# Rintazero/ft8_demodulator

Measured on AMD Instinct MI355X. Metric: 15-s FT8 slots/sec (full decode) + LDPC candidates/sec, 1/2/4/8 MI355X, higher is better.
Workload: dtype f32 (STFT, sync score) / f64 (LLR, BP); 1 GPU; BASELINE config 3: batch of 256 independent 15-s slots per GPU, 12 kHz, K=300 candidates, min_score=2, 20 BP iterations (config 5 shape at N>1); slots_per_gpu=256, max_candidates=300, min_score=2, pipeline_depth=2, parallelism=slot-sharded x1

## Files before the change

ft8_demodulator_amd/csrc/bp.hip:

```cpp
#include "ft8_internal.h"
#include "heap_replay.h"

namespace ft8 {
namespace {

__constant__ uint16_t kChkStartD[FT8_LDPC_M + 1] = FT8_CHK_START_INIT;
__constant__ uint8_t kEdgeVarD[FT8_LDPC_E] = FT8_EDGE_VAR_INIT;
__constant__ uint16_t kVarEdgeD[FT8_LDPC_N * 3] = FT8_VAR_EDGE_INIT;
__constant__ uint8_t kEdgeChkD[FT8_LDPC_E] = FT8_EDGE_CHK_INIT;
constexpr int kGrayD[8] = {0, 1, 3, 2, 5, 6, 4, 7};

constexpr int kEdgeSlots = (FT8_LDPC_E + kWave - 1) / kWave;
constexpr int kVarSlots = (FT8_LDPC_N + kWave - 1) / kWave;
constexpr int kChkSlots = (FT8_LDPC_M + kWave - 1) / kWave;

constexpr int kDivGroup = 3;
static_assert(kEdgeSlots % kDivGroup == 0 && kVarSlots == kDivGroup, "division groups tile the slots exactly");
constexpr int kBpWavesPerSimd = 4;
constexpr int kBpLbWaves = 3;
constexpr int kBpGridCus = 256;
constexpr double kClip2 = 2.0 * 4.97;

typedef __attribute__((address_space(3))) const double lds_f64;
typedef __attribute__((address_space(3))) const uint64_t lds_u64;

__device__ double sqrt_rn(double x) {
  double y = __builtin_sqrt(x);
  if (!(x > 0.0) || __builtin_isinf(x)) return y;
  for (int it = 0; it < 4; ++it) {
    const double lo = __longlong_as_double(__double_as_longlong(y) - 1);
    const double hi = __longlong_as_double(__double_as_longlong(y) + 1);
    if (__builtin_fma(y, lo, -x) >= 0.0) { y = lo; continue; }
    if (__builtin_fma(y, hi, -x) < 0.0) { y = hi; continue; }
    break;
  }
  return y;
}

__device__ __forceinline__ double pymax4(double a, double b, double c, double d) {
  double m = a;
  m = b > m ? b : m;
  m = c > m ? c : m;
  m = d > m ? d : m;
  return m;
}

template <int N>
__device__ __forceinline__ void div_fast(double* q, const double* x, const double* y) {
  double r[N], e[N], m[N];
#pragma unroll
  for (int i = 0; i < N; ++i) r[i] = __builtin_amdgcn_rcp(y[i]);
#pragma unroll
  for (int i = 0; i < N; ++i) e[i] = __builtin_fma(-y[i], r[i], 1.0);
#pragma unroll
  for (int i = 0; i < N; ++i) r[i] = __builtin_fma(r[i], e[i], r[i]);
#pragma unroll
  for (int i = 0; i < N; ++i) e[i] = __builtin_fma(-y[i], r[i], 1.0);
#pragma unroll
  for (int i = 0; i < N; ++i) r[i] = __builtin_fma(r[i], e[i], r[i]);
#pragma unroll
  for (int i = 0; i < N; ++i) m[i] = x[i] * r[i];
#pragma unroll
  for (int i = 0; i < N; ++i) e[i] = __builtin_fma(-y[i], m[i], x[i]);
#pragma unroll
  for (int i = 0; i < N; ++i) q[i] = __builtin_fma(e[i], r[i], m[i]);
}

template <int N, bool NEG2 = false>
__device__ __forceinline__ void div_rn(double* q, const double* x, const double* y_in, int fast = 0) {
  int ok = fast;
  if (!ok) {
    double mn = __builtin_fabs(x[0]);
#pragma unroll
    for (int i = 1; i < N; ++i) mn = __builtin_fmin(mn, __builtin_fabs(x[i]));
    ok = __ballot(mn >= 0x1p-960) == __builtin_amdgcn_read_exec() ? 1 : 0;
  }
  double r[N], e[N], m[N];
  if (ok) {
#pragma unroll
    for (int i = 0; i < N; ++i) r[i] = __builtin_amdgcn_rcp(y_in[i]);
#pragma unroll
    for (int i = 0; i < N; ++i) e[i] = __builtin_fma(-y_in[i], r[i], 1.0);
#pragma unroll
    for (int i = 0; i < N; ++i) r[i] = __builtin_fma(r[i], e[i], r[i]);
#pragma unroll
    for (int i = 0; i < N; ++i) e[i] = __builtin_fma(-y_in[i], r[i], 1.0);
#pragma unroll
    for (int i = 0; i < N; ++i) r[i] = __builtin_fma(r[i], e[i], r[i]);
#pragma unroll
    for (int i = 0; i < N; ++i) m[i] = x[i] * r[i];
#pragma unroll
    for (int i = 0; i < N; ++i) e[i] = __builtin_fma(-y_in[i], m[i], x[i]);
#pragma unroll
    for (int i = 0; i < N; ++i) q[i] = __builtin_fma(e[i], r[i], m[i]);
    return;
  }
  double den[N], num[N], y[N];
  bool f0[N], f1[N];
#pragma unroll
  for (int i = 0; i < N; ++i) y[i] = NEG2 ? -2.0 * y_in[i] : y_in[i];
#pragma unroll
  for (int i = 0; i < N; ++i) den[i] = __builtin_amdgcn_div_scale(x[i], y[i], false, &f0[i]);
#pragma unroll
  for (int i = 0; i < N; ++i) r[i] = __builtin_amdgcn_rcp(den[i]);
#pragma unroll
  for (int i = 0; i < N; ++i) num[i] = __builtin_amdgcn_div_scale(x[i], y[i], true, &f1[i]);
#pragma unroll
  for (int i = 0; i < N; ++i) e[i] = __builtin_fma(-den[i], r[i], 1.0);
#pragma unroll
  for (int i = 0; i < N; ++i) r[i] = __builtin_fma(r[i], e[i], r[i]);
#pragma unroll
  for (int i = 0; i < N; ++i) e[i] = __builtin_fma(-den[i], r[i], 1.0);
#pragma unroll
  for (int i = 0; i < N; ++i) r[i] = __builtin_fma(r[i], e[i], r[i]);
#pragma unroll
  for (int i = 0; i < N; ++i) m[i] = num[i] * r[i];
#pragma unroll
  for (int i = 0; i < N; ++i) e[i] = __builtin_fma(-den[i], m[i], num[i]);
#pragma unroll
  for (int i = 0; i < N; ++i) q[i] = __builtin_amdgcn_div_fmas(e[i], r[i], m[i], f1[i]);
#pragma unroll
  for (int i = 0; i < N; ++i) q[i] = __builtin_amdgcn_div_fixup(q[i], y[i], x[i]);
  if constexpr (NEG2) {
#pragma unroll
    for (int i = 0; i < N; ++i) q[i] = -2.0 * q[i];
  }
  (void)f0;
}

constexpr int kM7 = 24;
constexpr int kQS = FT8_LDPC_M;
constexpr int kQ6 = 6 * kQS;
constexpr int kMsgN = 584;
constexpr int kOne = kMsgN - 1;
constexpr int kHdr = 1024;
static_assert(kEdgeSlots * kWave <= kMsgN && kQ6 + kM7 == FT8_LDPC_E, "row-major message layout");

constexpr int kLeftRows = FT8_LDPC_M - kWave;
constexpr int kLeftLanes = 3 * kLeftRows;
constexpr int kRowB = 8 * kQS;
static_assert(kWave + kLeftRows == FT8_LDPC_M && kLeftRows == 19, "64 + 19 rows");
static_assert(kM7 <= kWave, "every leftover row has degree 6");
static_assert(kLeftLanes <= kWave, "3 x 19 leftover lanes fit the wave");
static_assert(kQ6 + kWave - 1 < kMsgN, "a check-major lane's seventh factor is a message or a constant");
static_assert(kEdgeSlots == 7 + 2, "seven check-major products and two leftover ones per lane");
__host__ __device__ constexpr int left_q3(int lane) { return lane / kLeftRows < 3 ? lane / kLeftRows : 2; }
__host__ __device__ constexpr int left_r(int lane) { return lane % kLeftRows; }
__host__ __device__ constexpr int left_f0(int q3) { return q3 == 0 ? 1 : 0; }
__host__ __device__ constexpr int left_f1(int q3) { return q3 == 2 ? 1 : 2; }
__host__ __device__ constexpr int msg_idx(int q, int mp) { return q * kQS + mp; }
__host__ __device__ constexpr bool phase_d_mapping_ok() {
  int stores[kMsgN] = {};
  for (int lane = 0; lane < kWave; ++lane) {
    for (int f = 0; f < 7; ++f) {
      if (msg_idx(f, lane) >= kMsgN) return false;
      if (f < 6 || lane < kM7) stores[msg_idx(f, lane)]++;
    }
    const int q3 = left_q3(lane), row = kWave + left_r(lane);
    for (int s = 0; s < 2; ++s) {
      const int fs[5] = {3 * s + left_f0(q3), 3 * s + left_f1(q3), 3 * (1 - s), 3 * (1 - s) + 1, 3 * (1 - s) + 2};
      int seen = 0;
      for (int k = 0; k < 5; ++k) {
        if (fs[k] < 0 || fs[k] > 5 || row >= FT8_LDPC_M || msg_idx(fs[k], row) >= kQ6) return false;
        seen |= 1 << fs[k];
      }
      if (seen != (0x3f & ~(1 << (3 * s + q3)))) return false;
      if (lane < kLeftLanes) stores[msg_idx(3 * s + q3, row)]++;
    }
  }
  for (int x = 0; x < kMsgN; ++x)
    if (stores[x] != (x < FT8_LDPC_E ? 1 : 0)) return false;
  return true;
}
static_assert(phase_d_mapping_ok(), "phase D reads inside msg and produces every edge exactly once");

struct WaveLds {
  uint8_t bits[256];
  uint8_t a91[16];
  uint8_t rank[FT8_LDPC_M];
  uint8_t chk_of[FT8_LDPC_M];
  uint8_t pad_[kHdr - 256 - 16 - 2 * FT8_LDPC_M];
  double msg[kMsgN];
};
static_assert(offsetof(WaveLds, msg) == kHdr, "msg follows the header");

struct WaveTables {
  uint32_t va[kVarSlots], va1[kVarSlots];
  uint32_t vb[kVarSlots];
  uint32_t h[kChkSlots][kVarSlots][2];
};

__device__ __forceinline__ double ldv(uint32_t addr) {
  return *(const volatile __attribute__((address_space(3))) double*)(uintptr_t)addr;
}

__device__ __forceinline__ uint32_t lds_addr(const void* p) {
  return (uint32_t)(uintptr_t)(__attribute__((address_space(3))) const void*)p;
}

__device__ void load_tables(WaveTables& t, WaveLds& L, int lane) {
  if (lane == 0) {
    int c7 = 0, c6 = kM7;
    for (int m = 0; m < FT8_LDPC_M; ++m) {
      const int r = (kChkStartD[m + 1] - kChkStartD[m]) == 7 ? c7++ : c6++;
      L.rank[m] = (uint8_t)r;
      L.chk_of[r] = (uint8_t)m;
    }
  }
  __syncthreads();
  const uint32_t msg0 = lds_addr(&L.msg[0]);
  auto addr_of = [&](int e) -> uint32_t {
    const int m = kEdgeChkD[e], q = e - kChkStartD[m], r = L.rank[m];
    return msg0 + 8u * (uint32_t)(q < 6 ? q * kQS + r : kQ6 + r);
  };
#pragma unroll
  for (int j = 0; j < kVarSlots; ++j) {
    const int n = lane + kWave * j;
    if (n < FT8_LDPC_N) {
      t.va[j] = addr_of(kVarEdgeD[3 * n]);
      t.va1[j] = addr_of(kVarEdgeD[3 * n + 1]);
      t.vb[j] = addr_of(kVarEdgeD[3 * n + 2]);
    } else {
      const uint32_t one = msg0 + 8u * kOne;
      t.va[j] = t.va1[j] = one;
      t.vb[j] = one;
    }
  }
#pragma unroll
  for (int k = 0; k < kChkSlots; ++k) {
    const int mp = lane + kWave * k;
#pragma unroll
    for (int j = 0; j < kVarSlots; ++j) t.h[k][j][0] = t.h[k][j][1] = 0;
    if (mp < FT8_LDPC_M) {
      const int m = L.chk_of[mp];
      for (int e = kChkStartD[m]; e < kChkStartD[m + 1]; ++e) {
        const int v = kEdgeVarD[e];
#pragma unroll
        for (int j = 0; j < kVarSlots; ++j)
#pragma unroll
          for (int w = 0; w < 2; ++w)
            if (v >> 5 == 2 * j + w) t.h[k][j][w] |= 1u << (v & 31);
      }
    }
  }
  for (int x = FT8_LDPC_E + lane; x < kMsgN; x += kWave) L.msg[x] = 1.0;
  __syncthreads();
#pragma unroll
  for (int j = 0; j < kVarSlots; ++j) asm volatile("" : "+v"(t.va[j]), "+v"(t.vb[j]));
#pragma unroll
  for (int j = 0; j < kVarSlots; ++j) asm volatile("" : "+v"(t.va1[j]));
#pragma unroll
  for (int k = 0; k < kChkSlots; ++k)
#pragma unroll
    for (int j = 0; j < kVarSlots; ++j) asm volatile("" : "+v"(t.h[k][j][0]), "+v"(t.h[k][j][1]));
}

struct BpArgs {
  const void* wf;
  int wf_f64, T, F, sps, bpt, num_blocks;
  const int32_t* cand;
  const double* cand_score;
  const int32_t* cand_count;
  int N, n_items, mode, n_slots;
  const double* llr_in;
  int normalize, max_iterations;
  double* llr_out;
  uint8_t* plain_out;
  ft8_result* res;
  unsigned long long* work;
  unsigned long long work_base;
  unsigned long long* stats;
  unsigned long long* clock;
  int slot0;
  int tie_blocks;
  TieArgs tie;
};

__device__ bool tie_order(const TieArgs& a, int slot) {
  if (slot >= a.n_slots) return false;
  const int w = a.warn[slot];
  if (!(w & 8)) return false;
  const int lane = threadIdx.x, N = a.N;
  const int nsel = __builtin_amdgcn_readfirstlane(a.cand_count[slot]);
  int32_t* t = a.tie + (int64_t)slot * tie_stride(N);
  const int32_t* push = t;
  const int32_t* sel = t + N;
  int32_t* perm = t + 2 * N;
  int32_t* mi = t + 3 * N;
  int32_t* mp = t + 4 * N;
  int32_t* mk = t + 5 * N;
  const int rec = t[7 * N];
  const float* psc = reinterpret_cast<const float*>(t + 7 * N + 2);
  const double* ssc = a.cand_score + (int64_t)slot * N;
  unsigned hh[kReplayRegs], hl[kReplayRegs];
  heap_load(psc, push, nsel, hh, hl);
  int tie = heap_pushes(nsel, hh, hl);
  if (rec >= 0) tie |= heap_record(nsel, hh, hl, mono_neg(__int_as_float(t[7 * N + 1])), (unsigned)rec);

  int M = 0;
  for (int i0 = 0; i0 < nsel; i0 += kWave) {
    const int i = i0 + lane;
    unsigned key = 0, idx = 0;
    bool mem = false;
    if (i < nsel) {
      idx = (unsigned)sel[i];
      key = mono_neg((float)ssc[i]);
      mem = (i > 0 && mono_neg((float)ssc[i - 1]) == key) || (i + 1 < nsel && mono_neg((float)ssc[i + 1]) == key);
    }
    unsigned long long b = __ballot(mem);
    while (b) {
      const int l = __ffsll((long long)b) - 1;
      b &= b - 1;
      const unsigned sl = rdl(idx, l), kl = rdl(key, l);
      unsigned P = 0;
#pragma unroll
      for (int k = 0; k < kReplayRegs; ++k) {
        const int pos = 64 * k + lane;
        const unsigned long long m = __ballot(pos >= 1 && pos <= nsel && hl[k] == sl);
        if (m) P = 64u * k + (unsigned)(__ffsll((long long)m) - 1);
      }
      if (lane == 0) {
        mi[M] = i0 + l;
        mp[M] = (int)P;
        mk[M] = (int)kl;
      }
      ++M;
    }
  }
  for (int i = lane; i < nsel; i += kWave) perm[i] = i;
  __syncthreads();
  for (int m = lane; m < M; m += kWave) {
    const int i = mi[m], P = mp[m], K = mk[m];
    int below_i = 0, below_p = 0;
    for (int j = 0; j < M; ++j) {
      if (mk[j] == K) {
        below_i += mi[j] < i;
        below_p += mp[j] < P;
      }
    }
    perm[i - below_i + below_p] = i;
  }
  if (lane == 0 && tie) a.warn[slot] = w | 1;
  return true;
}

__global__ __launch_bounds__(kWave) void k_tie_apply(TieArgs a, int32_t* cand, double* cand_score) {
  const int slot = blockIdx.x, lane = threadIdx.x, N = a.N;
  if (!tie_order(a, slot)) return;
  __syncthreads();
  const int nsel = a.cand_count[slot];
  int32_t* t = a.tie + (int64_t)slot * tie_stride(N);
  const int32_t* perm = t + 2 * N;
  int32_t* stage = t + 3 * N;
  int32_t* cs = cand + (int64_t)slot * N * 2;
  double* ss = cand_score + (int64_t)slot * N;
  for (int i = lane; i < nsel; i += kWave) {
    const int src = perm[i];
    stage[4 * i] = cs[2 * src];
    stage[4 * i + 1] = cs[2 * src + 1];
    const long long v = __double_as_longlong(ss[src]);
    stage[4 * i + 2] = (int32_t)v;
    stage[4 * i + 3] = (int32_t)(v >> 32);
  }
  __syncthreads();
  for (int i = lane; i < nsel; i += kWave) {
    cs[2 * i] = stage[4 * i];
    cs[2 * i + 1] = stage[4 * i + 1];
    ss[i] = __longlong_as_double(((long long)stage[4 * i + 3] << 32) | (unsigned)stage[4 * i + 2]);
  }
}

constexpr int kLlrCpw = 4;
constexpr int kLlrRow = FT8_LDPC_N + 2;

__device__ double pairwise174x4(const double (*x)[kLlrRow], double (*part)[16], int lane) {
  const int u = lane >> 4, l = lane & 15;
  const double* xu = x[u];
  double r;
  if (l < 8) {
    r = xu[l];
    for (int i = 8; i < 80; i += 8) r += xu[i + l];
  } else {
    const int j = l - 8;
    r = xu[80 + j];
    for (int i = 8; i < 88; i += 8) r += xu[80 + i + j];
  }
  part[u][l] = r;
  __syncthreads();
  double tot = 0.0;
  if (l == 0) {
    const double* pu = part[u];
    const double s1 = ((pu[0] + pu[1]) + (pu[2] + pu[3])) + ((pu[4] + pu[5]) + (pu[6] + pu[7]));
    double s2 = ((pu[8] + pu[9]) + (pu[10] + pu[11])) + ((pu[12] + pu[13]) + (pu[14] + pu[15]));
    for (int i = 168; i < 174; ++i) s2 += xu[i];
    tot = 0.0 + (s1 + s2);
  }
  __syncthreads();
  return __shfl(tot, lane & ~15);
}

template <typename T>
__device__ void extract_llr_x4(const BpArgs& a, const int (&slot)[kLlrCpw], const int (&at)[kLlrCpw],
                               const int (&af)[kLlrCpw], int n_on, double (*c)[kLlrRow], T (*stage)[64 * 8],
                               int lane) {
  const int i = lane & 7, g = lane >> 3;
  const T* wf0 = reinterpret_cast<const T*>(a.wf);
  T v[kLlrCpw][8];
#pragma unroll
  for (int u = 0; u < kLlrCpw; ++u) {
    const int base = floordiv(at[u], a.sps);
    const T* wf = wf0 + (int64_t)slot[u] * a.T * a.F;
#pragma unroll
    for (int r = 0; r < 8; ++r) {
      const int k = 8 * r + g;
      const int sym = k + (k < 29 ? 7 : 14);
      const int block = base + sym;
      v[u][r] = (T)0;
      if (u < n_on && k < 58 && !(block < 0 || block >= a.num_blocks))
        v[u][r] = wf[(int64_t)(at[u] + sym * a.sps) * a.F + af[u] + i * a.bpt];
    }
  }
#pragma unroll
  for (int u = 0; u < kLlrCpw; ++u)
#pragma unroll
    for (int r = 0; r < 8; ++r) stage[u][8 * (8 * r + g) + i] = v[u][r];
  __syncthreads();
  if (lane < 58) {
    const int k = lane;
    const int sym = k + (k < 29 ? 7 : 14);
#pragma unroll
    for (int u = 0; u < kLlrCpw; ++u) {
      if (u >= n_on) break;
      const int block = floordiv(at[u], a.sps) + sym;
      double l0 = 0.0, l1 = 0.0, l2 = 0.0;
      if (!(block < 0 || block >= a.num_blocks)) {
        double s[8], s2[8];
#pragma unroll
        for (int j = 0; j < 8; ++j) s[j] = (double)stage[u][8 * k + j];
#pragma unroll
        for (int j = 0; j < 8; ++j) s2[j] = s[kGrayD[j]];
        l0 = pymax4(s2[4], s2[5], s2[6], s2[7]) - pymax4(s2[0], s2[1], s2[2], s2[3]);
        l1 = pymax4(s2[2], s2[3], s2[6], s2[7]) - pymax4(s2[0], s2[1], s2[4], s2[5]);
        l2 = pymax4(s2[1], s2[3], s2[5], s2[7]) - pymax4(s2[0], s2[2], s2[4], s2[6]);
      }
      c[u][3 * k] = l0;
      c[u][3 * k + 1] = l1;
      c[u][3 * k + 2] = l2;
    }
  }
}

template <typename T>
__global__ __launch_bounds__(kWave) void k_llr(BpArgs a) {
  __shared__ double c[kLlrCpw][kLlrRow];
  __shared__ double part[kLlrCpw][16];
  __shared__ double bc[kLlrCpw];
  constexpr size_t kScratch = sizeof(T) * kLlrCpw * 64 * 8 > sizeof(double) * kLlrCpw * kLlrRow
                                  ? sizeof(T) * kLlrCpw * 64 * 8 : sizeof(double) * kLlrCpw * kLlrRow;
  __shared__ __attribute__((aligned(16))) unsigned char scratch[kScratch];
  double (*sq)[kLlrRow] = reinterpret_cast<double (*)[kLlrRow]>(scratch);
  const int lane = threadIdx.x;
  if ((int)blockIdx.x < a.tie_blocks) {
    tie_order(a.tie, blockIdx.x);
    return;
  }
  const int id = blockIdx.x - a.tie_blocks;
  int item0, n_on;
  int slot[kLlrCpw] = {0, 0, 0, 0}, at[kLlrCpw] = {0, 0, 0, 0}, af[kLlrCpw] = {0, 0, 0, 0};
  static_assert(kLlrCpw == 4, "four candidates per wave");
  if (a.mode == 0) {
    const int groups = (a.N + kLlrCpw - 1) / kLlrCpw;
    const int q = id >> 3;
    const int s0 = (q / groups) * 8 + (id & 7);
    const int c0 = (q % groups) * kLlrCpw;
    if (s0 >= a.n_slots) return;
    n_on = min(kLlrCpw, min(a.N, a.cand_count[s0]) - c0);
    item0 = s0 * a.N + c0;
#pragma unroll
    for (int u = 0; u < kLlrCpw; ++u) {
      slot[u] = s0;
      if (u < n_on) {
        at[u] = a.cand[((int64_t)item0 + u) * 2];
        af[u] = a.cand[((int64_t)item0 + u) * 2 + 1];
      }
    }
  } else {
    item0 = id * kLlrCpw;
    n_on = min(kLlrCpw, a.n_items - item0);
    if (a.mode == 1) {
#pragma unroll
      for (int u = 0; u < kLlrCpw; ++u) {
        if (u < n_on) {
          slot[u] = a.cand[((int64_t)item0 + u) * 3];
          at[u] = a.cand[((int64_t)item0 + u) * 3 + 1];
          af[u] = a.cand[((int64_t)item0 + u) * 3 + 2];
        }
      }
    }
  }
  if (n_on <= 0) return;
  if (a.mode == 2) {
    for (int e = lane; e < n_on * FT8_LDPC_N; e += kWave) {
      const int u = e / FT8_LDPC_N, n = e - u * FT8_LDPC_N;
      c[u][n] = a.llr_in[(int64_t)(item0 + u) * FT8_LDPC_N + n];
    }
  } else {
    extract_llr_x4<T>(a, slot, at, af, n_on, c, reinterpret_cast<T (*)[64 * 8]>(scratch), lane);
  }
  __syncthreads();
  if (a.normalize) {
    const double mean = pairwise174x4(c, part, lane) / 174.0;
    if ((lane & 15) == 0) bc[lane >> 4] = mean;
    __syncthreads();
    for (int e = lane; e < n_on * FT8_LDPC_N; e += kWave) {
      const int u = e / FT8_LDPC_N, n = e - u * FT8_LDPC_N;
      const double d = c[u][n] - bc[u];
      sq[u][n] = d * d;
    }
    __syncthreads();
    const double var = pairwise174x4(sq, part, lane) / 174.0;
    if ((lane & 15) == 0) bc[lane >> 4] = sqrt_rn(24.0 / var);
    __syncthreads();
    for (int e = lane; e < n_on * FT8_LDPC_N; e += kWave) {
      const int u = e / FT8_LDPC_N, n = e - u * FT8_LDPC_N;
      a.llr_out[(int64_t)(item0 + u) * FT8_LDPC_N + n] = c[u][n] * bc[u];
    }
    return;
  }
  for (int e = lane; e < n_on * FT8_LDPC_N; e += kWave) {
    const int u = e / FT8_LDPC_N, n = e - u * FT8_LDPC_N;
    a.llr_out[(int64_t)(item0 + u) * FT8_LDPC_N + n] = c[u][n];
  }
}

__device__ __forceinline__ void sweep_sync() { asm volatile("" ::: "memory"); }

__device__ __forceinline__ double clip2(double T, bool nan_in) {
  const double y = __builtin_fmin(__builtin_fmax(T, -kClip2), kClip2);
  return (nan_in && T != T) ? T : y;
}

__device__ __forceinline__ void tanh_group(double* v, int fast = 0) {
  double na[kDivGroup], nb[kDivGroup];
#pragma unroll
  for (int i = 0; i < kDivGroup; ++i) {
    const double yv = v[i], z = yv * yv;
    na[i] = yv * (15120.0 + z * (420.0 + z));
    nb[i] = -30240.0 + z * (-3360.0 + z * -30.0);
  }
  int ok = fast;
  if (!ok) {
    double mn = INFINITY;
#pragma unroll
    for (int i = 0; i < kDivGroup; ++i) mn = __builtin_fmin(mn, __builtin_fabs(na[i]));
    ok = __ballot(mn >= 0x1p-480) == __builtin_amdgcn_read_exec() ? 1 : 0;
  }
  if (ok) {
    div_fast<kDivGroup>(v, na, nb);
  } else {
#pragma unroll
    for (int i = 0; i < kDivGroup; ++i) {
      const double xv = -0.5 * v[i], x2 = xv * xv;
      na[i] = xv * (945.0 + x2 * (105.0 + x2));
      nb[i] = 945.0 + x2 * (420.0 + x2 * 15.0);
    }
    div_rn<kDivGroup>(v, na, nb);
  }
}

__device__ __forceinline__ float min3_abs_hi(double a, double b, double c) {
  float m;
  asm("v_min3_f32 %0, |%1|, |%2|, |%3|"
      : "=v"(m)
      : "v"(__double2hiint(a)), "v"(__double2hiint(b)), "v"(__double2hiint(c)));
  return m;
}

__device__ __forceinline__ bool sweep_fast(const double (&y)[kVarSlots][3]) {
  static_assert(kVarSlots == 3, "three variable slots");
  const float m0 = min3_abs_hi(y[0][0], y[0][1], y[0][2]);
  const float m1 = min3_abs_hi(y[1][0], y[1][1], y[1][2]);
  const float m2 = min3_abs_hi(y[2][0], y[2][1], y[2][2]);
  float m;
  asm("v_min3_f32 %0, %1, %2, %3" : "=v"(m) : "v"(m0), "v"(m1), "v"(m2));
  const float thr = __int_as_float(923 << 20);
  return __ballot(m < thr) == 0;
}

__device__ __forceinline__ void atanh_group(double* v, int fast = 0) {
  double na[kDivGroup], nb[kDivGroup];
#pragma unroll
  for (int i = 0; i < kDivGroup; ++i) {
    const double xv = v[i], x2 = xv * xv;
    na[i] = xv * (945.0 + x2 * __builtin_fma(x2, 64.0, -735.0));
    nb[i] = (-472.5 + x2 * (525.0 + x2 * -112.5));
  }
  div_rn<kDivGroup, true>(v, na, nb, fast);
}

struct LeftAddr {
  uint32_t rb, f0, f1, st;
};

__device__ __forceinline__ LeftAddr left_addr(uint32_t msg0, int lane) {
  const int q3 = left_q3(lane);
  LeftAddr a;
  a.rb = msg0 + 8u * (uint32_t)(kWave + left_r(lane));
  a.f0 = a.rb + (uint32_t)(kRowB * left_f0(q3));
  a.f1 = a.rb + (uint32_t)(kRowB * left_f1(q3));
  a.st = a.rb + (uint32_t)(kRowB * q3);
  return a;
}

__device__ __forceinline__ void row_products(double* x, uint32_t la) {
  double t[7];
#pragma unroll
  for (int f = 0; f < 7; ++f) t[f] = ldv(la + (uint32_t)(kRowB * f));
  double p = t[1];
#pragma unroll
  for (int f = 2; f < 7; ++f) p *= t[f];
  x[0] = p;
  double pre = t[0];
#pragma unroll
  for (int q = 1; q < 7; ++q) {
    p = pre;
#pragma unroll
    for (int f = q + 1; f < 7; ++f) p *= t[f];
    x[q] = p;
    pre *= t[q];
  }
}

__device__ __forceinline__ void left_products(double* x, const LeftAddr& a) {
  double p = ldv(a.f0) * ldv(a.f1);
#pragma unroll
  for (int f = 3; f < 6; ++f) p *= ldv(a.rb + (uint32_t)(kRowB * f));
  x[0] = p;
  p = ldv(a.rb);
#pragma unroll
  for (int f = 1; f < 3; ++f) p *= ldv(a.rb + (uint32_t)(kRowB * f));
  p *= ldv(a.f0 + (uint32_t)(kRowB * 3));
  p *= ldv(a.f1 + (uint32_t)(kRowB * 3));
  x[1] = p;
}

template <bool NANSAFE>
__global__ __launch_bounds__(kWave, kBpLbWaves) void k_bp(BpArgs a) {
  const unsigned long long clk0 = a.clock ? clock64() : 0ull, wall0 = a.clock ? wall_clock64() : 0ull;
  __shared__ WaveLds L;
  const int lane = threadIdx.x;
  WaveTables tb;
  load_tables(tb, L, lane);
  const bool var2 = lane + kWave * (kVarSlots - 1) < FT8_LDPC_N;
  const uint64_t var2_mask = (1ull << (FT8_LDPC_N - kWave * (kVarSlots - 1))) - 1ull;
  uint32_t la = lds_addr(&L.msg[0]) + 8u * (uint32_t)lane;
  asm volatile("" : "+v"(la));
  LeftAddr lf = left_addr(la - 8u * (uint32_t)lane, lane);
  asm volatile("" : "+v"(lf.rb), "+v"(lf.f0), "+v"(lf.f1), "+v"(lf.st));

  unsigned st_cand = 0, st_iter = 0, st_pass = 0, st_conv = 0;
  for (;;) {
    unsigned long long ticket = 0;
    if (lane == 0) ticket = atomicAdd(a.work, 1ull);
    const unsigned lo = __builtin_amdgcn_readfirstlane((unsigned)ticket);
    const unsigned hi = __builtin_amdgcn_readfirstlane((unsigned)(ticket >> 32));
    const unsigned long long rel = (((unsigned long long)hi << 32) | lo) - a.work_base;
    if (rel >= (unsigned long long)a.n_items) break;
    const unsigned item = (unsigned)rel;

    int slot = 0, at = 0, af = 0, cidx = 0;
    double score = 0.0;
    if (a.mode == 0) {
      slot = item / a.N;
      cidx = item % a.N;
      if (cidx >= a.cand_count[slot]) continue;
      at = a.cand[((int64_t)slot * a.N + cidx) * 2];
      af = a.cand[((int64_t)slot * a.N + cidx) * 2 + 1];
      score = a.cand_score[(int64_t)slot * a.N + cidx];
    }
    double cv_[kVarSlots];
#pragma unroll
    for (int j = 0; j < kVarSlots; ++j) {
      const int n = lane + kWave * j;
      cv_[j] = n < FT8_LDPC_N ? a.llr_in[(int64_t)item * FT8_LDPC_N + n] : -1.0;
    }

    const bool nan_in = NANSAFE && __ballot(cv_[0] != cv_[0] || cv_[1] != cv_[1] || cv_[2] != cv_[2]) != 0;

#pragma unroll
    for (int i = 0; i < kEdgeSlots; ++i)
      if (i < kEdgeSlots - 1 || lane + kWave * i < FT8_LDPC_E)
        *(__attribute__((address_space(3))) double*)(uintptr_t)(la + 512u * i) = 0.0;
    __syncthreads();
    uint64_t hd[kVarSlots] = {0, 0, 0};
    int min_errors = FT8_LDPC_M;
    int entered = 0, passes = 0;
    for (int iter = 0; iter < a.max_iterations; ++iter) {
      entered++;
#pragma unroll
      for (int j = 0; j < kVarSlots; ++j) asm volatile("" : "+v"(tb.va[j]), "+v"(tb.vb[j]));
      double y[kVarSlots][3];
      const bool sweep0 = iter == 0;
      if (sweep0) {
#pragma unroll
        for (int j = 0; j < kVarSlots; ++j) {
          const double T = cv_[j] + 0.0;
          hd[j] = __ballot(T > 0.0);
          y[j][0] = y[j][1] = y[j][2] = clip2(T, nan_in);
        }
      } else {
#pragma unroll
        for (int j = 0; j < kVarSlots; ++j) {
          const double t0 = *(lds_f64*)(uintptr_t)tb.va[j];
          const double t1 = *(lds_f64*)(uintptr_t)tb.va1[j];
          const double t2 = *(lds_f64*)(uintptr_t)tb.vb[j];
          const double c = cv_[j];
          hd[j] = __ballot((c + ((t0 + t1) + t2)) > 0.0);
          const double c0 = c + t0;
          y[j][0] = (c + t1) + t2;
          y[j][1] = c0 + t2;
          y[j][2] = c0 + t1;
        }
        if (nan_in) {
#pragma unroll
          for (int j = 0; j < kVarSlots; ++j)
#pragma unroll
            for (int e = 0; e < 3; ++e) y[j][e] = clip2(y[j][e], true);
        } else {
#pragma unroll
          for (int j = 0; j < kVarSlots; ++j)
#pragma unroll
            for (int e = 0; e < 3; ++e) y[j][e] = clip2(y[j][e], false);
        }
      }
      hd[kVarSlots - 1] &= var2_mask;
      if ((hd[0] | hd[1] | hd[2]) == 0) break;
      int errs = 0;
#pragma unroll
      for (int k = 0; k < kChkSlots; ++k) {
        uint32_t x = 0;
#pragma unroll
        for (int j = 0; j < kVarSlots; ++j) {
          x = __builtin_amdgcn_bitop3_b32(tb.h[k][j][0], (uint32_t)hd[j], x, 0x6a);
          x = __builtin_amdgcn_bitop3_b32(tb.h[k][j][1], (uint32_t)(hd[j] >> 32), x, 0x6a);
        }
        errs += __popcll(__ballot(__builtin_popcount(x) & 1));
      }
      if (errs < min_errors) {
        min_errors = errs;
        if (errs == 0) break;
      }
      if (iter + 1 == a.max_iterations) break;
      static_assert(kDivGroup == 3 && kVarSlots == 3, "a division group is one variable's edges");
      int fast = __builtin_amdgcn_readfirstlane(sweep_fast(y) ? 1 : 0);
      asm volatile("" : "+s"(fast));
      if (sweep0) {
        double v[kVarSlots] = {y[0][0], y[1][0], y[2][0]};
        tanh_group(v, fast);
#pragma unroll
        for (int j = 0; j < kVarSlots; ++j) y[j][0] = y[j][1] = y[j][2] = v[j];
      }
#pragma unroll
      for (int j = 0; j < kVarSlots; ++j) {
        if (!sweep0) tanh_group(y[j], fast);
        if (j < kVarSlots - 1 || var2) {
          *(__attribute__((address_space(3))) double*)(uintptr_t)tb.va[j] = y[j][0];
          *(__attribute__((address_space(3))) double*)(uintptr_t)tb.va1[j] = y[j][1];
          *(__attribute__((address_space(3))) double*)(uintptr_t)tb.vb[j] = y[j][2];
        }
        asm volatile("" ::: "memory");
      }
      sweep_sync();
      double x[kEdgeSlots];
      row_products(x, la);
      left_products(&x[7], lf);
#pragma unroll
      for (int g = 0; g < kEdgeSlots; g += kDivGroup) atanh_group(&x[g], fast);
#pragma unroll
      for (int f = 0; f < 6; ++f)
        *(__attribute__((address_space(3))) double*)(uintptr_t)(la + (uint32_t)(kRowB * f)) = x[f];
      if (lane < kM7)
        *(__attribute__((address_space(3))) double*)(uintptr_t)(la + (uint32_t)(kRowB * 6)) = x[6];
      if (lane < kLeftLanes) {
        *(__attribute__((address_space(3))) double*)(uintptr_t)lf.st = x[7];
        *(__attribute__((address_space(3))) double*)(uintptr_t)(lf.st + (uint32_t)(kRowB * 3)) = x[8];
      }
      passes++;
      sweep_sync();
    }
    const bool pack = a.res && min_errors == 0;
    if (a.plain_out || pack) {
#pragma unroll
      for (int j = 0; j < kVarSlots; ++j) L.bits[lane + kWave * j] = (uint8_t)((hd[j] >> lane) & 1u);
      __syncthreads();
    }
    st_cand++;
    st_iter += entered;
    st_pass += passes;
    st_conv += min_errors == 0;


    if (a.plain_out)
      for (int n = lane; n < FT8_LDPC_N; n += kWave) a.plain_out[(int64_t)item * FT8_LDPC_N + n] = L.bits[n];
    if (a.res) {
      if (pack && lane < 12) {
        const uint64_t w = *reinterpret_cast<const uint64_t*>(&L.bits[8 * lane]);
        const uint32_t lo = (uint32_t)w, hi = (uint32_t)(w >> 32);
        unsigned byte = 0;
#pragma unroll
        for (int j = 0; j < 4; ++j) byte |= ((lo >> (8 * j)) & 1u) << (7 - j);
#pragma unroll
        for (int j = 0; j < 4; ++j) byte |= ((hi >> (8 * j)) & 1u) << (3 - j);
        if (lane == 11) byte &= 0xE0u;
        L.a91[lane] = (uint8_t)byte;
      }
      __syncthreads();
      if (lane == 0) {
        ft8_result r;
        r.score = score;
        r.slot = a.slot0 + slot;
        r.abs_time = at;
        r.abs_freq = af;
        r.ldpc_errors = (int16_t)min_errors;
        r.cand_index = (uint16_t)cidx;
        r.crc_extracted = 0;
        r.crc_calculated = 0;
        r.ok = 0;
        r.pass_index = 0;
        for (int i = 0; i < 10; ++i) r.payload[i] = 0;
        if (min_errors == 0) {
          const uint8_t* a91 = L.a91;
          const unsigned ce = ((a91[9] & 7u) << 11) | ((unsigned)a91[10] << 3) | (a91[11] >> 5);
          uint8_t buf[12];
          for (int i = 0; i < 10; ++i) buf[i] = a91[i];
          buf[9] &= 0xF8;
          buf[10] = 0;
          buf[11] = 0;
          unsigned rem = 0;
          for (int ib = 0; ib < 82; ++ib) {
            if ((ib & 7) == 0) rem ^= (unsigned)buf[ib >> 3] << 6;
            rem = (rem & 0x2000u) ? ((rem << 1) ^ 0x2757u) : (rem << 1);
          }
          const unsigned cc = rem & 0x3FFFu;
          r.crc_extracted = (uint16_t)ce;
          r.crc_calculated = (uint16_t)cc;
          if (ce == cc) {
            r.ok = 1;
            for (int i = 0; i < 10; ++i) r.payload[i] = a91[i];
            r.payload[9] &= 0xF8;
          }
        }
        a.res[item] = r;
      }
    }
    __syncthreads();
  }
  const unsigned row = (blockIdx.x & (unsigned)(kStatRows - 1)) * (unsigned)kStatStride;
  if (a.stats && lane == 0 && st_cand) {
    atomicAdd(&a.stats[row + 0], (unsigned long long)st_cand);
    atomicAdd(&a.stats[row + 1], (unsigned long long)st_iter);
    atomicAdd(&a.stats[row + 2], (unsigned long long)st_pass);
    atomicAdd(&a.stats[row + 3], (unsigned long long)st_conv);
  }
  if (a.clock && lane == 0) {
    const unsigned long long cyc = clock64() - clk0, wall = wall_clock64() - wall0;
    atomicAdd(&a.clock[row + 0], cyc);
    atomicAdd(&a.clock[row + 1], wall);
    atomicMax(&a.clock[row + 2], cyc);
    atomicAdd(&a.clock[row + 3], 1ull);
  }
}

__global__ __launch_bounds__(kWave) void k_compact(const ft8_result* res, const int32_t* cand_count,
                                                   int N, ft8_result* out, int32_t* counts, int cap,
                                                   const int32_t* warn, const int32_t* tie) {
  const int slot = blockIdx.x, lane = threadIdx.x;
  const int nc = cand_count[slot];
  const int32_t* perm = (tie && (warn[slot] & 8)) ? tie + (int64_t)slot * tie_stride(N) + 2 * N : nullptr;
  const ft8_result* rs = res + (int64_t)slot * N;
  int base = 0;
  for (int c0 = 0; c0 < nc; c0 += kWave) {
    const int c = c0 + lane;
    const int src = c < nc ? (perm ? perm[c] : c) : 0;
    const bool ok = c < nc && rs[src].ok;
    const unsigned long long m = __ballot(ok);
    const int pos = base + __popcll(m & ((1ull << lane) - 1ull));
    if (ok && pos < cap) {
      out[(int64_t)slot * cap + pos] = rs[src];
      if (perm) out[(int64_t)slot * cap + pos].cand_index = (uint16_t)c;
    }
    base += __popcll(m);
  }
  if (lane == 0) counts[slot] = base;
}

constexpr int kPackThreads = 1024;
__global__ __launch_bounds__(kPackThreads) void k_pack(const ft8_result* rec, const int32_t* counts, int n_slots,
                                                       int cap, int capacity, int slot_offset, uint8_t* send,
                                                       ft8_result* overflow) {
  FT8_RACE_PROLOGUE();
  __shared__ int s_off[kPackThreads];
  __shared__ int s_wave[kPackThreads / kWave + 1];
  const int tid = threadIdx.x, lane = tid & (kWave - 1), w = tid >> 6;
  int32_t* cnt_out = reinterpret_cast<int32_t*>(send + 8);
  ft8_result* rows = reinterpret_cast<ft8_result*>(send + pack_header_bytes(n_slots));
  int carry = 0;
  for (int base = 0; base < n_slots; base += kPackThreads) {
    const int s = base + tid;
    int c = 0;
    if (s < n_slots) {
      const int raw = counts[s];
      cnt_out[s] = raw;
      c = min(max(raw, 0), cap);
    }
    int x = c;
#pragma unroll
    for (int o = 1; o < kWave; o <<= 1) {
      const int y = __shfl_up(x, o);
      if (lane >= o) x += y;
    }
    if (lane == kWave - 1) s_wave[w] = x;
    __syncthreads();
    if (tid == 0) {
      int acc = 0;
      for (int i = 0; i < kPackThreads / kWave; ++i) {
        const int t = s_wave[i];
        s_wave[i] = acc;
        acc += t;
      }
      s_wave[kPackThreads / kWave] = acc;
    }
    __syncthreads();
    s_off[tid] = s < n_slots ? s_wave[w] + x - c : 0x7fffffff;
    const int ct = s_wave[kPackThreads / kWave];
    __syncthreads();
    for (int r = tid; r < ct; r += kPackThreads) {
      int lo = 0, hi = min(kPackThreads, n_slots - base) - 1;
      while (lo < hi) {
        const int mid = (lo + hi + 1) >> 1;
        if (s_off[mid] <= r) lo = mid;
        else hi = mid - 1;
      }
      ft8_result v = rec[(int64_t)(base + lo) * cap + (r - s_off[lo])];
      v.slot += slot_offset;
      const int dst = carry + r;
      if (dst < capacity) rows[dst] = v;
      else if (overflow) overflow[dst - capacity] = v;
    }
    carry += ct;
    __syncthreads();
  }
  for (int r = carry + tid; r < capacity; r += kPackThreads) {
    uint64_t* p = reinterpret_cast<uint64_t*>(rows + r);
#pragma unroll
    for (int i = 0; i < (int)(sizeof(ft8_result) / 8); ++i) p[i] = 0;
  }
  for (int i = n_slots + tid; i < (int)((pack_header_bytes(n_slots) - 8) / 4); i += kPackThreads) cnt_out[i] = 0;
  if (tid == 0) *reinterpret_cast<int64_t*>(send) = carry;
}

__global__ void k_crc14(const uint8_t* msg, const int32_t* nbits, int n, uint16_t* crc) {
  const int i = blockIdx.x * blockDim.x + threadIdx.x;
  if (i >= n) return;
  const uint8_t* m = msg + (int64_t)i * 12;
  const int nb = nbits[i];
  unsigned rem = 0;
  for (int b = 0; b < nb; ++b) {
    if ((b & 7) == 0) rem ^= (unsigned)m[b >> 3] << 6;
    rem = (rem & 0x2000u) ? ((rem << 1) ^ 0x2757u) : (rem << 1);
  }
  crc[i] = (uint16_t)(rem & 0x3FFFu);
}

__global__ void k_ldpc_check(const uint8_t* bits, int n, int32_t* err) {
  const int i = blockIdx.x * blockDim.x + threadIdx.x;
  if (i >= n) return;
  const uint8_t* b = bits + (int64_t)i * FT8_LDPC_N;
  int e = 0;
  for (int m = 0; m < FT8_LDPC_M; ++m) {
    int x = 0;
    for (int j = kChkStartD[m]; j < kChkStartD[m + 1]; ++j) x ^= b[kEdgeVarD[j]];
    e += x != 0;
  }
  err[i] = e;
}

BpArgs make_args(const BpLaunch& L) {
  BpArgs a{};
  a.wf = L.wf;
  a.wf_f64 = L.wf_f64;
  a.T = L.T;
  a.F = L.F;
  a.sps = L.sps;
  a.bpt = L.bpt;
  a.num_blocks = L.sps > 0 ? L.T / L.sps : 0;
  a.cand = L.cand;
  a.cand_score = L.cand_score;
  a.cand_count = L.cand_count;
  a.N = L.N;
  a.n_items = L.n_items;
  a.n_slots = L.n_slots;
  a.mode = L.mode;
  a.llr_in = L.llr_in;
  a.normalize = L.normalize;
  a.max_iterations = L.max_iterations;
  a.llr_out = L.llr_out;
  a.plain_out = L.plain_out;
  a.res = L.res;
  a.work = L.work;
  a.work_base = L.work_base ? *L.work_base : 0ull;
  a.stats = L.stats;
  a.clock = L.clock;
  a.slot0 = L.slot0;
  a.tie = TieArgs{L.n_slots, L.N, L.cand_count, L.warn, L.tie, L.cand_score};
  a.tie_blocks = (L.tie && L.mode == 0) ? (L.n_slots + 7) / 8 * 8 : 0;
  return a;
}

}

hipError_t launch_llr(const BpLaunch& L, hipStream_t s) {
  if (L.n_items <= 0) return hipSuccess;
  BpArgs a = make_args(L);
  const int64_t grid = a.tie_blocks + (L.mode == 0 ? (int64_t)((L.n_slots + 7) / 8) * 8 * ((L.N + kLlrCpw - 1) / kLlrCpw)
                                                    : ((int64_t)L.n_items + kLlrCpw - 1) / kLlrCpw);
  if (L.wf_f64)
    hipLaunchKernelGGL(k_llr<double>, dim3((unsigned)grid), dim3(kWave), 0, s, a);
  else
    hipLaunchKernelGGL(k_llr<float>, dim3((unsigned)grid), dim3(kWave), 0, s, a);
  return hipGetLastError();
}

hipError_t launch_bp(const BpLaunch& L, hipStream_t s) {
  if (L.n_items <= 0) return hipSuccess;
  BpArgs a = make_args(L);
  const int per_simd = max(1, min(L.grid_waves, kBpWavesPerSimd));
  const int waves = min(L.n_items, kBpGridCus * 4 * per_simd);
  if (L.mode == 0) hipLaunchKernelGGL(k_bp<false>, dim3(waves), dim3(kWave), 0, s, a);
  else hipLaunchKernelGGL(k_bp<true>, dim3(waves), dim3(kWave), 0, s, a);
  const hipError_t e = hipGetLastError();
  if (e == hipSuccess && L.work_base) *L.work_base += (unsigned long long)L.n_items + (unsigned long long)waves;
  return e;
}

hipError_t launch_tie_apply(const TieArgs& a, int32_t* cand, double* cand_score, hipStream_t s) {
  if (a.n_slots <= 0 || !a.tie) return hipSuccess;
  hipLaunchKernelGGL(k_tie_apply, dim3(a.n_slots), dim3(kWave), 0, s, a, cand, cand_score);
  return hipGetLastError();
}

hipError_t launch_compact(const CompactLaunch& L, hipStream_t s) {
  if (L.n_slots <= 0) return hipSuccess;
  hipLaunchKernelGGL(k_compact, dim3(L.n_slots), dim3(kWave), 0, s, L.res, L.cand_count, L.N, L.out,
                     L.counts, L.cap, L.warn, L.tie);
  return hipGetLastError();
}

hipError_t launch_pack(const ft8_result* rec, const int32_t* counts, int n_slots, int cap, int capacity,
                       int slot_offset, uint8_t* send, ft8_result* overflow, hipStream_t s) {
  static_assert(sizeof(ft8_result) % 8 == 0, "records are copied as 8-byte words");
  hipLaunchKernelGGL(k_pack, dim3(1), dim3(kPackThreads), 0, s, rec, counts, n_slots, cap, capacity, slot_offset,
                     send, overflow);
  return hipGetLastError();
}

hipError_t launch_crc14(const uint8_t* msg, const int32_t* nbits, int n, uint16_t* crc, hipStream_t s) {
  if (n <= 0) return hipSuccess;
  hipLaunchKernelGGL(k_crc14, dim3((n + 255) / 256), dim3(256), 0, s, msg, nbits, n, crc);
  return hipGetLastError();
}

hipError_t launch_ldpc_check(const uint8_t* bits, int n, int32_t* err, hipStream_t s) {
  if (n <= 0) return hipSuccess;
  hipLaunchKernelGGL(k_ldpc_check, dim3((n + 255) / 256), dim3(256), 0, s, bits, n, err);
  return hipGetLastError();
}

}
```

Before: 148,300 slots/s.

## Peel first BP sweep, split fast/slow atanh paths with rescaled rational constants

```diff
diff --git a/ft8_demodulator_amd/csrc/bp.hip b/ft8_demodulator_amd/csrc/bp.hip
--- a/ft8_demodulator_amd/csrc/bp.hip
+++ b/ft8_demodulator_amd/csrc/bp.hip
@@ -1,5 +1,7 @@
 #include "ft8_internal.h"
 #include "heap_replay.h"
+
+#include <type_traits>
 
 namespace ft8 {
 namespace {
@@ -67,34 +69,15 @@
 }
 
 template <int N, bool NEG2 = false>
-__device__ __forceinline__ void div_rn(double* q, const double* x, const double* y_in, int fast = 0) {
-  int ok = fast;
-  if (!ok) {
-    double mn = __builtin_fabs(x[0]);
-#pragma unroll
-    for (int i = 1; i < N; ++i) mn = __builtin_fmin(mn, __builtin_fabs(x[i]));
-    ok = __ballot(mn >= 0x1p-960) == __builtin_amdgcn_read_exec() ? 1 : 0;
+__device__ __forceinline__ void div_rn(double* q, const double* x, const double* y_in) {
+  double mn = __builtin_fabs(x[0]);
+#pragma unroll
+  for (int i = 1; i < N; ++i) mn = __builtin_fmin(mn, __builtin_fabs(x[i]));
+  if (__ballot(mn >= 0x1p-960) == __builtin_amdgcn_read_exec()) {
+    div_fast<N>(q, x, y_in);
+    return;
   }
   double r[N], e[N], m[N];
-  if (ok) {
-#pragma unroll
-    for (int i = 0; i < N; ++i) r[i] = __builtin_amdgcn_rcp(y_in[i]);
-#pragma unroll
-    for (int i = 0; i < N; ++i) e[i] = __builtin_fma(-y_in[i], r[i], 1.0);
-#pragma unroll
-    for (int i = 0; i < N; ++i) r[i] = __builtin_fma(r[i], e[i], r[i]);
-#pragma unroll
-    for (int i = 0; i < N; ++i) e[i] = __builtin_fma(-y_in[i], r[i], 1.0);
-#pragma unroll
-    for (int i = 0; i < N; ++i) r[i] = __builtin_fma(r[i], e[i], r[i]);
-#pragma unroll
-    for (int i = 0; i < N; ++i) m[i] = x[i] * r[i];
-#pragma unroll
-    for (int i = 0; i < N; ++i) e[i] = __builtin_fma(-y_in[i], m[i], x[i]);
-#pragma unroll
-    for (int i = 0; i < N; ++i) q[i] = __builtin_fma(e[i], r[i], m[i]);
-    return;
-  }
   double den[N], num[N], y[N];
   bool f0[N], f1[N];
 #pragma unroll
@@ -587,7 +570,27 @@
   return __ballot(m < thr) == 0;
 }
 
-__device__ __forceinline__ void atanh_group(double* v, int fast = 0) {
+constexpr double kAt1 = -735.0 / 64.0;
+constexpr double kAt2 = 945.0 / 64.0;
+constexpr double kAt3 = -472.5 / 64.0;
+constexpr double kAt4 = 525.0 / 64.0;
+constexpr double kAt5 = -112.5 / 64.0;
+static_assert(64.0 * kAt1 == -735.0 && 64.0 * kAt2 == 945.0, "numerator constants are exact / 64");
+static_assert(64.0 * kAt3 == -472.5 && 64.0 * kAt4 == 525.0 && 64.0 * kAt5 == -112.5,
+              "denominator constants are exact / 64");
+
+__device__ __forceinline__ void atanh_group_fast(double* v) {
+  double na[kDivGroup], nb[kDivGroup];
+#pragma unroll
+  for (int i = 0; i < kDivGroup; ++i) {
+    const double xv = v[i], x2 = xv * xv;
+    na[i] = xv * (x2 * (x2 + kAt1) + kAt2);
+    nb[i] = kAt3 + x2 * (kAt4 + x2 * kAt5);
+  }
+  div_fast<kDivGroup>(v, na, nb);
+}
+
+__device__ __forceinline__ void atanh_group(double* v) {
   double na[kDivGroup], nb[kDivGroup];
 #pragma unroll
   for (int i = 0; i < kDivGroup; ++i) {
@@ -595,7 +598,7 @@
     na[i] = xv * (945.0 + x2 * __builtin_fma(x2, 64.0, -735.0));
     nb[i] = (-472.5 + x2 * (525.0 + x2 * -112.5));
   }
-  div_rn<kDivGroup, true>(v, na, nb, fast);
+  div_rn<kDivGroup, true>(v, na, nb);
 }
 
 struct LeftAddr {
@@ -656,6 +659,7 @@
   uint32_t la = lds_addr(&L.msg[0]) + 8u * (uint32_t)lane;
   asm volatile("" : "+v"(la));
   LeftAddr lf = left_addr(la - 8u * (uint32_t)lane, lane);
+  int lane_v = lane;
   asm volatile("" : "+v"(lf.rb), "+v"(lf.f0), "+v"(lf.f1), "+v"(lf.st));
 
   unsigned st_cand = 0, st_iter = 0, st_pass = 0, st_conv = 0;
@@ -695,13 +699,13 @@
     uint64_t hd[kVarSlots] = {0, 0, 0};
     int min_errors = FT8_LDPC_M;
     int entered = 0, passes = 0;
-    for (int iter = 0; iter < a.max_iterations; ++iter) {
+    auto sweep = [&](auto first, int iter) __attribute__((always_inline)) -> bool {
+      constexpr bool sweep0 = decltype(first)::value;
       entered++;
 #pragma unroll
       for (int j = 0; j < kVarSlots; ++j) asm volatile("" : "+v"(tb.va[j]), "+v"(tb.vb[j]));
       double y[kVarSlots][3];
-      const bool sweep0 = iter == 0;
-      if (sweep0) {
+      if constexpr (sweep0) {
 #pragma unroll
         for (int j = 0; j < kVarSlots; ++j) {
           const double T = cv_[j] + 0.0;
@@ -715,7 +719,7 @@
           const double t1 = *(lds_f64*)(uintptr_t)tb.va1[j];
           const double t2 = *(lds_f64*)(uintptr_t)tb.vb[j];
           const double c = cv_[j];
-          hd[j] = __ballot((c + ((t0 + t1) + t2)) > 0.0);
+          hd[j] = __ballot(((t0 + t1) + t2) > -c);
           const double c0 = c + t0;
           y[j][0] = (c + t1) + t2;
           y[j][1] = c0 + t2;
@@ -734,7 +738,7 @@
         }
       }
       hd[kVarSlots - 1] &= var2_mask;
-      if ((hd[0] | hd[1] | hd[2]) == 0) break;
+      if ((hd[0] | hd[1] | hd[2]) == 0) return true;
       int errs = 0;
 #pragma unroll
       for (int k = 0; k < kChkSlots; ++k) {
@@ -748,9 +752,9 @@
       }
       if (errs < min_errors) {
         min_errors = errs;
-        if (errs == 0) break;
-      }
-      if (iter + 1 == a.max_iterations) break;
+        if (errs == 0) return true;
+      }
+      if (iter + 1 == a.max_iterations) return true;
       static_assert(kDivGroup == 3 && kVarSlots == 3, "a division group is one variable's edges");
       int fast = __builtin_amdgcn_readfirstlane(sweep_fast(y) ? 1 : 0);
       asm volatile("" : "+s"(fast));
@@ -774,20 +778,30 @@
       double x[kEdgeSlots];
       row_products(x, la);
       left_products(&x[7], lf);
-#pragma unroll
-      for (int g = 0; g < kEdgeSlots; g += kDivGroup) atanh_group(&x[g], fast);
+      if (fast) {
+#pragma unroll
+        for (int g = 0; g < kEdgeSlots; g += kDivGroup) atanh_group_fast(&x[g]);
+      } else {
+#pragma unroll
+        for (int g = 0; g < kEdgeSlots; g += kDivGroup) atanh_group(&x[g]);
+      }
 #pragma unroll
       for (int f = 0; f < 6; ++f)
         *(__attribute__((address_space(3))) double*)(uintptr_t)(la + (uint32_t)(kRowB * f)) = x[f];
-      if (lane < kM7)
+      asm volatile("" : "+v"(lane_v));
+      if (lane_v < kM7)
         *(__attribute__((address_space(3))) double*)(uintptr_t)(la + (uint32_t)(kRowB * 6)) = x[6];
-      if (lane < kLeftLanes) {
+      if (lane_v < kLeftLanes) {
         *(__attribute__((address_space(3))) double*)(uintptr_t)lf.st = x[7];
         *(__attribute__((address_space(3))) double*)(uintptr_t)(lf.st + (uint32_t)(kRowB * 3)) = x[8];
       }
       passes++;
       sweep_sync();
-    }
+      return false;
+    };
+    if (a.max_iterations > 0 && !sweep(std::true_type{}, 0))
+      for (int iter = 1; iter < a.max_iterations; ++iter)
+        if (sweep(std::false_type{}, iter)) break;
     const bool pack = a.res && min_errors == 0;
     if (a.plain_out || pack) {
 #pragma unroll
```

Measured after the change: 148,200 slots/s. No clear change (-0.1%).
